# songlab-cal/CherryML

Measured on AMD Instinct MI355X. Metric: cherry-pairs/sec (whole node) per EM iter, higher is better.
Workload: dtype f64

## Files before the change

### cherryml_amd/csrc/cb_internal.hip.h

```cpp
#pragma once
#include "../../include/cherrybank.h"

#include <hip/hip_runtime.h>

#include <algorithm>
#include <atomic>
#include <chrono>
#include <cmath>
#include <cstdarg>
#include <cstdio>
#include <cstdlib>
#include <cstring>
#include <string>
#include <vector>

int cb_fail(int code, const char *fmt, ...);
#define fail cb_fail

#define HIP_TRY(expr)                                                                   \
  do {                                                                                  \
    hipError_t e_ = (expr);                                                             \
    if (e_ != hipSuccess)                                                               \
      return fail(e_ == hipErrorOutOfMemory ? CB_ENOMEM : CB_EHIP, "%s failed: %s (%s:%d)", \
                  #expr, hipGetErrorString(e_), __FILE__, __LINE__);                    \
  } while (0)

#define CB_REUSE_EIGH 256
int cb_internal_expm_bank(cb_handle h, const double *Q, const double *pi, int flags, double *P);
int cb_internal_set_times(cb_handle h, const double *t_host, int B, const double *t_dev);
struct CbSpectral {
  int S = 0, LD = 0;
  const double *A = nullptr, *U = nullptr, *lam = nullptr, *dsq = nullptr, *sigma = nullptr;
};
int cb_internal_spectral(cb_handle h, CbSpectral *out);

int cb_launch_bank_fused(int variant, int kg, const void *args, int grid, hipStream_t stream, hipEvent_t stop);

#define CB_TB_RS_MAX 24
#define CB_TB_RG_MAX 40
struct CbTimeBasisHost {
  int B = 0, ns = 0, nd = 0, ng = 0;
  double rho_max = 0.0;
  double res_s = 0.0, res_g = 0.0;
  std::vector<int> kind;
  std::vector<int> skel_s, direct, skel_g;
  std::vector<double> tf, tg;
  std::vector<double> Ls, Lg;
};
bool cb_tb_build(int B, const double *t, double rho_max, CbTimeBasisHost &out);
struct CbTbEwArgs {
  int S, LD, B, ns, nd, ng;
  int nsmall;
  const double *Ct;
  const double *Psi;
  const double *A;
  const double *t;
  const double *Ls, *Lg;
  double *Gh;
  float *Gh32;
  double *loss_part;
  double inv_n;
  const unsigned long long *skip;
};
int cb_tb_launch_tables(int LD, int ns, int nd, int ng, const double *tf, const double *tg, const double *lam, double *F, double *E,
                        double *H, const unsigned long long *skip, hipStream_t stream);
#define CB_TB_LDS_MAX (144u << 10)
size_t cb_tb_ew_lds_bytes(int B, int ns, int ng);
bool cb_tb_supported(int B, int LD, int ns, int ng);
int cb_tb_prepare_ew(int B, int ns, int ng, size_t *cache);
int cb_tb_launch_ew(const CbTbEwArgs &a, hipStream_t stream, hipEvent_t stop, int *nparts);

static inline const char *cb_test_hook(const char *name) {
  const char *on = getenv("CB_TEST_HOOKS");
  return (on && on[0] == '1') ? getenv(name) : nullptr;
}

struct CbDevBufs {
  std::vector<void *> ptrs;
  ~CbDevBufs() {
    for (void *p : ptrs)
      if (p) (void)hipFree(p);
  }
  template <typename T>
  T *up(const T *host, size_t count, int &rc) {
    void *q = nullptr;
    if (rc != CB_OK) return nullptr;
    if (hipMalloc(&q, (count ? count : 1) * sizeof(T)) != hipSuccess) {
      rc = fail(CB_ENOMEM, "device allocation failed");
      return nullptr;
    }
    ptrs.push_back(q);
    if (host && count && hipMemcpyAsync(q, host, count * sizeof(T), hipMemcpyHostToDevice, 0) != hipSuccess)
      rc = fail(CB_EHIP, "upload failed");
    return static_cast<T *>(q);
  }
};

struct __attribute__((visibility("hidden"))) CbKernelTimer {
  const bool on, owned;
  hipEvent_t ev0 = nullptr, ev1 = nullptr;
  explicit CbKernelTimer(bool on_) : on(on_), owned(true) {}
  CbKernelTimer(bool on_, hipEvent_t b0, hipEvent_t b1) : on(on_), owned(false), ev0(b0), ev1(b1) {}
  CbKernelTimer(const CbKernelTimer &) = delete;
  ~CbKernelTimer() { drop(); }
  void drop() {
    if (owned && ev0) (void)hipEventDestroy(ev0);
    if (owned && ev1) (void)hipEventDestroy(ev1);
    ev0 = ev1 = nullptr;
  }
  int create() {
    HIP_TRY(hipEventCreate(&ev0));
    HIP_TRY(hipEventCreate(&ev1));
    return CB_OK;
  }
  int begin(bool sync_first) {
    if (!on) return CB_OK;
    const int rc = owned ? create() : CB_OK;
    if (rc != CB_OK) return rc;
    if (sync_first) HIP_TRY(hipStreamSynchronize(0));
    HIP_TRY(hipEventRecord(ev0, 0));
    return CB_OK;
  }
  int end(double *ms) {
    if (!on) return CB_OK;
    float t = 0.f;
    HIP_TRY(hipEventRecord(ev1, 0));
    HIP_TRY(hipEventSynchronize(ev1));
    HIP_TRY(hipEventElapsedTime(&t, ev0, ev1));
    *ms = t;
    drop();
    return CB_OK;
  }
};
```

### cherryml_amd/csrc/cherrybank.hip

```cpp
#include "cb_internal.hip.h"

#include "common.hip.h"
#include "jacobi_block.hip.h"
#include "jacobi_wave.hip.h"
#include "large_bank.hip.h"
#include "small_bank.hip.h"
#include "train_small.hip.h"
#include "train_large.hip.h"
#include "general_small.hip.h"
#include "general_large.hip.h"
#include "eigh_planned.hip.h"

#define CB_ABI_VERSION 2

static thread_local std::string g_err;

int cb_fail(int code, const char *fmt, ...) {
  char buf[512];
  va_list ap;
  va_start(ap, fmt);
  vsnprintf(buf, sizeof buf, fmt, ap);
  va_end(ap);
  g_err = buf;
  return code;
// ... 131 lines not shown
static double tb_growth() {
  if (const char *g = cb_test_hook("CB_TB_TEST_GROWTH")) return std::max(1.0, atof(g));
  return CB_TB_GROWTH;
}
static void tb_drop_next(cb_bank *h) {
  if (h->tb_next_pending) (void)h->tb_next.get();
  h->tb_next_pending = false;
}
static int tb_install(cb_bank *h, int B, CbTimeBasisHost &&nb, double ms) {
  if (nb.B != B || !cb_tb_supported(B, h->LD, nb.ns, nb.ng) || (h->dtype == CB_MIXED && 2 * (nb.ns + nb.nd) > B) ||
      cb_tb_prepare_ew(B, nb.ns, nb.ng, h->tb_ew_lds) != 0) {
    h->tb_failed = true;
    h->tb = CbTimeBasisHost{};
    return CB_OK;
  }
  const int set = h->tb_set ^ 1;
  HIP_TRY(hipMemcpy(h->tb_Ls[set], nb.Ls.data(), nb.Ls.size() * sizeof(double), hipMemcpyHostToDevice));
  HIP_TRY(hipMemcpy(h->tb_Lg[set], nb.Lg.data(), nb.Lg.size() * sizeof(double), hipMemcpyHostToDevice));
  HIP_TRY(hipMemcpy(h->tb_tf[set], nb.tf.data(), nb.tf.size() * sizeof(double), hipMemcpyHostToDevice));
  HIP_TRY(hipMemcpy(h->tb_tg[set], nb.tg.data(), nb.tg.size() * sizeof(double), hipMemcpyHostToDevice));
  h->tb = std::move(nb);
  h->tb_set = set;
  ++h->tb_builds;
  if (getenv("CB_DEBUG"))
    fprintf(stderr, "[cherrybank] time basis %d: rho_max %.3f, %d skeleton + %d direct forward, %d gradient buckets of %d; residuals %.1e / %.1e; %.1f ms%s\n",
            h->tb_builds, h->tb.rho_max, h->tb.ns, h->tb.nd, h->tb.ng, B, h->tb.res_s, h->tb.res_g, ms, ms < 0.0 ? " (built beside the epochs)" : "");
  return CB_OK;
}
static int tb_rebuild(cb_bank *h, int B, double two_sigma) {
  if (!(two_sigma > 0.0) || !std::isfinite(two_sigma)) return fail(CB_ENUMERIC, "time basis: max |Q_ii| = %g", 0.5 * two_sigma);
  tb_drop_next(h);
  const auto t0 = std::chrono::steady_clock::now();
  CbTimeBasisHost nb;
  if (!cb_tb_build(B, h->t_live_host.data(), two_sigma * tb_growth(), nb)) nb = CbTimeBasisHost{};
  HIP_TRY(hipStreamSynchronize(h->stream));
  return tb_install(h, B, std::move(nb), std::chrono::duration<double, std::milli>(std::chrono::steady_clock::now() - t0).count());
}
#ifndef CB_TB_LEAD
#define CB_TB_LEAD 64
#endif
static int tb_maintain(cb_bank *h, int B, int epoch, double two_sigma, bool stale) {
  if (cb_test_hook("CB_TB_TEST_GROWTH")) {
    if (stale) return tb_rebuild(h, B, two_sigma);
    return CB_OK;
  }
  if (h->tb_failed) return CB_OK;
  if (stale || !tb_in_range(h, B, two_sigma)) {
    bool took = false;
    if (h->tb_next_pending) {
      CbTimeBasisHost nb = h->tb_next.get();
      h->tb_next_pending = false;
      int rc = tb_install(h, B, std::move(nb), -1.0);
      if (rc != CB_OK || h->tb_failed) return rc;
      took = true;
    }
    if ((stale && !took) || !tb_in_range(h, B, two_sigma)) return tb_rebuild(h, B, two_sigma);
    return CB_OK;
  }
  double warn = 1.6;
  int lead = CB_TB_LEAD;
  if (const char *w = cb_test_hook("CB_TB_TEST_WARN")) sscanf(w, "%lf %d", &warn, &lead);
  if (h->tb_next_pending && epoch >= h->tb_next_epoch) {
    CbTimeBasisHost nb = h->tb_next.get();
    h->tb_next_pending = false;
    int rc = tb_install(h, B, std::move(nb), -1.0);
    if (rc != CB_OK || h->tb_failed) return rc;
  }
  if (!h->tb_next_pending && !tb_in_range(h, B, two_sigma, warn)) {
    std::vector<double> t(h->t_live_host.begin(), h->t_live_host.begin() + B);
    const double rho = two_sigma * tb_growth();
    h->tb_next = std::async(std::launch::async, [t, rho, B]() {
      CbTimeBasisHost nb;
      if (!cb_tb_build(B, t.data(), rho, nb)) nb = CbTimeBasisHost{};
      return nb;
    });
    h->tb_next_pending = true;
    h->tb_next_epoch = epoch + lead;
  }
  return CB_OK;
}

struct LargeBankForm {
  bool tb = false;
  bool fused = false;
  bool accum = false;
  int kg = 1;
  int n_parts = 1;
  int tiles_k3 = 0;
  int test_no_claim = 0;
  double phi_delta = 0;
};

static LargeBankForm choose_large_form(const cb_bank *h, int B, bool Pd, bool want_grad, bool planned_now) {
  static const int streams = getenv("CB_BANK_STREAMS") ? std::min(4, std::max(1, atoi(getenv("CB_BANK_STREAMS")))) : 1;
  const char *tb_hook = cb_test_hook("CB_BANK_TB"), *fused_hook = cb_test_hook("CB_BANK_FUSED"),
             *unfused_hook = cb_test_hook("CB_BANK_UNFUSED"), *k3_hook = cb_test_hook("CB_BANK_K3"),
             *kg_hook = cb_test_hook("CB_BANK_KG"), *no_claim_hook = cb_test_hook("CB_BANK_TEST_NO_CLAIM"),
             *phi_z_hook = cb_test_hook("CB_PHI_Z");
  const int LD = h->LD, tm = (LD + LG_TM - 1) / LG_TM, tn = (LD + LG_TN - 1) / LG_TN;
  const bool f32 = h->dtype == CB_F32 && !Pd;
  LargeBankForm f;
  const bool form_hooks = fused_hook || unfused_hook || k3_hook || kg_hook || no_claim_hook;
  f.tb = h->sym_counts && !h->per_bucket_products && !h->tb_block && !h->tb_failed && !Pd && want_grad && h->tb_Ls[0] &&
         streams == 1 && (h->dtype == CB_F64 || h->dtype == CB_MIXED) &&
         (tb_hook ? atoi(tb_hook) != 0 : (!form_hooks && B >= CB_TB_MIN_B));
  if (f.tb && planned_now && h->tb.B != B) f.tb = false;
  {
    const size_t nb16 = (size_t)LD / 16, cap = (size_t)B * tm * tn;
    if (nb16 * (nb16 + 1) > cap) f.tb = false;
  }
  f.fused = !Pd && want_grad && !unfused_hook && streams == 1 && h->bank_queue && (fused_hook || B >= CB_BANK_FUSED_MIN_B);
  f.accum = h->sym_counts && !h->per_bucket_products && !Pd && want_grad && h->Yk && streams == 1 && h->dtype == CB_F64 &&
            (k3_hook ? atoi(k3_hook) == 0 : (B >= CB_BANK_SUM_FIRST_MIN_B && h->phi_delta >= 4e-3));
  f.tiles_k3 = f.accum ? 0 : h->sym_counts ? tn * (tn + 1) / 2 : tm * tn;
  f.phi_delta = h->phi_delta;
  if (phi_z_hook) f.phi_delta *= atof(phi_z_hook) / 0.1;
  f.kg = (B < CB_BANK_KG2_MAX_B && !f32) ? 2 : 1;
  if (kg_hook) f.kg = atoi(kg_hook) == 1 ? 1 : 2;
  if (Pd) f.kg = 1;
  if (streams > 1 && h->dtype == CB_F64 && !Pd && want_grad && B >= 4 * streams && !h->comm && !h->profile) f.n_parts = streams;
  f.test_no_claim = no_claim_hook ? 1 : 0;
  return f;
}

struct LargeCall {
  int B;
  const double *t;
  double inv_n;
  double *loss, *dQ, *Pd;
  bool dA_padded, planned_now;
  const unsigned long long *skipw;
  size_t LL;
  int tiles, tiles_k1;
};

template <typename T1, typename TG>
struct BankBufs {
  const T1 *Ut, *A, *F, *Ct;
  TG *Gt, *T;
  const TG *U;
  int variant;
};
template <typename T1, typename TG>
static BankBufs<T1, TG> bank_bufs(const cb_bank *h) {
  if constexpr (std::is_same_v<T1, float>) return {h->Utf, h->Af, h->Ff, h->Ct32, h->Gt32, h->T32, h->Uf, 1};
  else if constexpr (std::is_same_v<TG, float>) return {h->Vc, h->A, h->F, h->Ct, h->Gt32, h->T32, h->Uf, 2};
  else return {h->Vc, h->A, h->F, h->Ct, h->Gt, h->T, h->U, 0};
}
template <typename Fn>
static int with_format(const cb_bank *h, bool Pd, Fn &&fn) {
  if (!Pd && h->dtype == CB_F32) return fn(float{}, float{});
  if (!Pd && h->dtype == CB_MIXED) return fn(double{}, float{});
  return fn(double{}, double{});
}

template <typename Args>
static void launch_kg(int kg, void (*kern1)(Args), void (*kern2)(Args), dim3 grid, hipStream_t st, hipEvent_t ev, const Args &a) {
  if (kg == 2) LAUNCH_STOP(ev, kern2, grid, dim3(2 * LG4_THREADS), 0, st, a);
  else LAUNCH_STOP(ev, kern1, grid, dim3(LG4_THREADS), 0, st, a);
}
static void launch_cast_f32(cb_bank *h, const LargeCall &c, size_t nF) {
  hipLaunchKernelGGL(lg_cast_f32, dim3((unsigned)((std::max(c.LL, nF) + 255) / 256)), dim3(256), 0, h->stream, c.LL, nF, h->U,
                     h->Vc, h->A, h->F, h->Uf, h->Utf, h->Af, h->Ff);
}
static void launch_tables(cb_bank *h, const LargeCall &c) {
  hipLaunchKernelGGL(lg_tables<NoBankArgs>, dim3((unsigned)(((size_t)c.B * h->LD + 255) / 256)), dim3(256), 0, h->stream, h->LD,
                     c.B, c.t, h->lam, h->sigma, h->F, h->E, h->H, NoBankArgs{}, (NoBankArgs *)nullptr, 0);
}

static void enqueue_k4(cb_bank *h, const LargeCall &c, const unsigned long long *skip, hipEvent_t stop) {
  const int S = h->S, LD = h->LD;
  K4Args k4a{S, LD, h->Mt, h->Vc, h->X, nullptr, nullptr, nullptr};
  k4a.skip = skip;
  launch_sg(h, k4a, 0);
  K4Args k4b{S, LD, h->Vc, h->X, c.dQ, c.dA_padded ? nullptr : h->dsq, nullptr, nullptr};
  k4b.skip = skip;
  launch_sg(h, k4b, 0, 0.0, 0.0, nullptr, stop);
}

template <typename TG>
static int enqueue_tail(cb_bank *h, const LargeBankForm &f, const LargeCall &c, const TG *src, int nb, int nparts, int sym_ld,
                        hipEvent_t k3_stop) {
  const int LD = h->LD;
  const LossArgs la{h->loss_part, nparts, h->S, h->dsq, h->dirsum, c.inv_n, c.loss, c.skipw};
  const dim3 red_grid((unsigned)((c.LL + 255) / 256) + 1);
  if (f.accum) {
    hipLaunchKernelGGL(ky_reduce_loss<TG>, red_grid, dim3(256), 0, h->stream, src, YArgs{LD, c.B, c.t, h->E, h->Yk}, la);
    K4Args gl{h->S, LD, h->Yk, h->U, h->Lk, nullptr, nullptr, nullptr};
    gl.skip = c.skipw;
    gl.ystride = c.LL;
    launch_sg(h, gl, 0, 0.0, 0.0, nullptr, nullptr, 1 + CB_PHI_TERMS);
    LAUNCH_STOP(k3_stop, kphi_combine<CB_PHI_TERMS>, dim3((unsigned)((c.LL + 255) / 256)), dim3(256), 0, h->stream, LD, h->Lk,
                h->lam, f.phi_delta, h->Mt, c.skipw);
  } else {
    hipLaunchKernelGGL(k3_reduce_loss<TG>, red_grid, dim3(256), 0, h->stream, src, nb, c.LL, h->Mt, sym_ld, la);
  }
  enqueue_k4(h, c, c.skipw, stop_event(h, EV_K4));
  HIP_TRY(hipGetLastError());
  return CB_OK;
}

template <typename TG>
static int enqueue_tb_bank(cb_bank *h, const LargeBankForm &f, const LargeCall &c) {
  constexpr bool mixed = std::is_same_v<TG, float>;
  const CbTimeBasisHost &bas = h->tb;
  const int S = h->S, LD = h->LD, set = h->tb_set, nf = bas.ns + bas.nd, ng = bas.ng;
  const auto bb = bank_bufs<double, TG>(h);
  if (!c.planned_now && cb_tb_launch_tables(LD, bas.ns, bas.nd, ng, h->tb_tf[set], h->tb_tg[set], h->lam, h->F, h->E, h->H,
                                            c.skipw, h->stream) != 0)
    return fail(CB_EHIP, "tb_tables: launch failed");
  double *psi_buf = mixed ? reinterpret_cast<double *>(h->T32) : h->T;
  K1Args<double> k1{S, LD, nf, h->Vc, h->A, h->tb_tf[set], h->F, h->sigma, h->Ct, psi_buf, h->loss_part, c.inv_n, h->dsq, nullptr, c.skipw};
  LAUNCH_STOP(stop_event(h, EV_K1), (k1_pt_loss_gt<double, double, false, 1, true>), dim3(c.tiles_k1 * nf), dim3(LG4_THREADS), 0,
              h->stream, k1);
  const CbTbEwArgs ew{S, LD, c.B, bas.ns, bas.nd, ng, c.B - bas.nd, h->Ct, psi_buf, h->A, c.t, h->tb_Ls[set], h->tb_Lg[set], h->Gt,
                      mixed ? h->Gt32 : nullptr, h->loss_part, c.inv_n, c.skipw};
  int ew_parts = 0;
  if (cb_tb_launch_ew(ew, h->stream, stop_event(h, EV_K2), &ew_parts) != 0) return fail(CB_EHIP, "tb_ew: launch failed");
  if (mixed) launch_cast_f32(h, c, 0);
  const K2Args<TG> k2{LD, bb.Gt, bb.U, bb.T, c.skipw};
  const K3Args<TG> k3{LD, ng, bb.T, bb.U, h->tb_tg[set], h->lam, h->E, h->H, bb.Gt, 1, c.skipw};
  hipLaunchKernelGGL((k2_t_eq_g_u<TG, 1>), dim3(c.tiles * ng), dim3(LG4_THREADS), 0, h->stream, k2);
  LAUNCH_STOP(stop_event(h, EV_K3), (k3_w_phi<TG, 1>), dim3(c.tiles_k1 * ng), dim3(LG4_THREADS), 0, h->stream, k3);
  return enqueue_tail<TG>(h, f, c, bb.Gt, ng, ew_parts, LD, nullptr);
}

template <typename T1, typename TG>
static int enqueue_fused_bank(cb_bank *h, const LargeBankForm &f, const LargeCall &c) {
  const int S = h->S, LD = h->LD, B = c.B;
  const auto bb = bank_bufs<T1, TG>(h);
  const int total = B * (c.tiles_k1 + c.tiles + f.tiles_k3), grid = std::min(h->bank_slots / f.kg, total);
  const int sym = h->sym_counts ? 1 : 0;
  if (h->profile && h->profile_now) h->ev_rec[EV_K1] = h->ev_rec[EV_K2] = false;
  const hipEvent_t bank_stop = stop_event(h, EV_K3);
  static_assert(sizeof(K123Args<float, float>) == sizeof(K123Args<double, double>) &&
                sizeof(K123Args<double, float>) == sizeof(K123Args<double, double>), "one argument block for all");
  const K123Args<T1, TG> a{{S, LD, B, bb.Ut, bb.A, c.t, bb.F, h->sigma, bb.Ct, bb.Gt, h->loss_part, c.inv_n, h->dsq, nullptr, c.skipw},
                           {LD, bb.Gt, bb.U, bb.T, c.skipw},
                           {LD, B, bb.T, bb.U, c.t, h->lam, h->E, h->H, bb.Gt, sym, c.skipw},
                           {h->bank_queue, B, c.tiles_k1, c.tiles, f.tiles_k3, h->bank_claims, f.test_no_claim}};
  auto *dst = reinterpret_cast<K123Args<T1, TG> *>(h->bank_args);
  hipLaunchKernelGGL((lg_tables<K123Args<T1, TG>>), dim3((unsigned)(((size_t)B * LD + 255) / 256)), dim3(256), 0, h->stream, LD, B,
                     c.t, h->lam, h->sigma, h->F, h->E, h->H, a, dst, grid);
  if (std::is_same_v<TG, float>) launch_cast_f32(h, c, (size_t)B * LD);
  if (cb_launch_bank_fused(bb.variant, f.kg, dst, grid, h->stream, bank_stop) != 0) return fail(CB_EHIP, "k123_bank: launch failed");
  return enqueue_tail<TG>(h, f, c, f.accum ? bb.T : bb.Gt, B, B * c.tiles_k1, h->sym_counts ? LD : 0, nullptr);
}

template <typename T1, typename TG>
static int enqueue_split_bank(cb_bank *h, const LargeBankForm &f, const LargeCall &c) {
  const int S = h->S, LD = h->LD, B = c.B;
  const auto bb = bank_bufs<T1, TG>(h);
  launch_tables(h, c);
  if (std::is_same_v<TG, float>) launch_cast_f32(h, c, (size_t)B * LD);
  const K1Args<T1, TG> k1{S, LD, B, bb.Ut, bb.A, c.t, bb.F, h->sigma, bb.Ct, bb.Gt, h->loss_part, c.inv_n, h->dsq, c.Pd, c.skipw};
  const hipEvent_t ev_k1 = stop_event(h, EV_K1);
  if constexpr (std::is_same_v<TG, double>) {
    if (c.Pd) {
      LAUNCH_STOP(ev_k1, (k1_pt_loss_gt<double, double, true>), dim3(c.tiles_k1 * B), dim3(LG4_THREADS), 0, h->stream, k1);
      HIP_TRY(hipGetLastError());
      return CB_OK;
    }
  }
  launch_kg(f.kg, k1_pt_loss_gt<T1, TG, false, 1>, k1_pt_loss_gt<T1, TG, false, 2>, dim3(c.tiles_k1 * B), h->stream, ev_k1, k1);
  if (!c.dQ) {
    hipLaunchKernelGGL(lg_finish_loss, dim3(1), dim3(256), 0, h->stream, h->loss_part, B * c.tiles_k1, S, h->dsq, h->dirsum,
                       c.inv_n, c.loss);
    HIP_TRY(hipGetLastError());
    return CB_OK;
  }
  const K2Args<TG> k2{LD, bb.Gt, bb.U, bb.T, c.skipw};
  launch_kg(f.kg, k2_t_eq_g_u<TG, 1>, k2_t_eq_g_u<TG, 2>, dim3(c.tiles * B), h->stream, stop_event(h, EV_K2), k2);
  const hipEvent_t ev_k3 = stop_event(h, EV_K3);
  if (f.accum) return enqueue_tail<TG>(h, f, c, bb.T, B, B * c.tiles_k1, 0, ev_k3);
  const K3Args<TG> k3{LD, B, bb.T, bb.U, c.t, h->lam, h->E, h->H, bb.Gt, h->sym_counts ? 1 : 0, c.skipw};
  launch_kg(f.kg, k3_w_phi<TG, 1>, k3_w_phi<TG, 2>, dim3(f.tiles_k3 * B), h->stream, ev_k3, k3);
  return enqueue_tail<TG>(h, f, c, bb.Gt, B, B * c.tiles_k1, h->sym_counts ? LD : 0, nullptr);
}

static int enqueue_stream_split_bank(cb_bank *h, const LargeBankForm &f, const LargeCall &c) {
  const int S = h->S, LD = h->LD, B = c.B, n = f.n_parts;
  const size_t LL = c.LL;
  launch_tables(h, c);
  if (!h->ev_fork) HIP_TRY(hipEventCreateWithFlags(&h->ev_fork, hipEventDisableTiming));
  for (int p = 1; p < n; ++p)
    if (!h->xstream[p - 1]) {
      HIP_TRY(hipStreamCreateWithFlags(&h->xstream[p - 1], hipStreamNonBlocking));
      HIP_TRY(hipEventCreateWithFlags(&h->ev_join[p - 1], hipEventDisableTiming));
    }
  HIP_TRY(hipEventRecord(h->ev_fork, h->stream));
  for (int p = 1; p < n; ++p) HIP_TRY(hipStreamWaitEvent(h->xstream[p - 1], h->ev_fork, 0));
  for (int k = 1; k <= 3; ++k)
    for (int p = 0; p < n; ++p) {
      const int b0 = (int)((long)B * p / n), Bs = (int)((long)B * (p + 1) / n) - b0;
      const hipStream_t st = p ? h->xstream[p - 1] : h->stream;
      double *Gt = h->Gt + b0 * LL, *T = h->T + b0 * LL;
      if (k == 1) {
        K1Args<double> k1{S, LD, Bs, h->Vc, h->A, c.t + b0, h->F + (size_t)b0 * LD, h->sigma, h->Ct + b0 * LL, Gt,
                          h->loss_part + (size_t)b0 * c.tiles_k1, c.inv_n, h->dsq, nullptr};
        launch_kg(f.kg, k1_pt_loss_gt<double, double, false, 1>, k1_pt_loss_gt<double, double, false, 2>, dim3(c.tiles_k1 * Bs),
                  st, nullptr, k1);
// ... 394 lines not shown
```

### cherryml_amd/csrc/handle_host.hip.h

```cpp
#pragma once
#include <hip/hip_ext.h>
#include <future>
struct EighSlot {
  int cap = 12;
  int nsq = 0;
  int band_after = 0;
  int so = 0;
  int expect_run = 1, expect_order = 12, expect_sq = 2;
};
struct EighPlan {
  int lead_band = 1;
  int nslots = 0;
  EighSlot slot[EC_MAXREC];
};
struct cb_bank {
  int dev = 0, S = 0, L = 0, B = 0;
  int B_cap = 0;
  hipStream_t xstream[3] = {};
  hipEvent_t ev_fork = nullptr, ev_join[3] = {};
  int tr_epochs = 0;
  uint64_t tr_sig = 0;
  int last_form = 0;
  double tr_pow_b1 = 1.0, tr_pow_b2 = 1.0;
  int dtype = CB_F64;
  int LD = 0;
  bool large = false;
  hipStream_t own_stream = nullptr, stream = nullptr;
  std::vector<void *> allocs;
  std::vector<double> n_host;
  double *t = nullptr;
  double *Ct = nullptr;
  double *n_dev = nullptr;
  double *inv_n = nullptr;
  double *ones = nullptr;
  double *Cq = nullptr;
  int nq = 0;
  double *dirsum = nullptr;
  double *dirsum_g = nullptr;
  int Bl = 0;
  double *t_live = nullptr;
  int *nlive = nullptr;
  std::vector<int> nlive_host;
  double *Q = nullptr, *pi = nullptr, *loss = nullptr, *dQ = nullptr;
  int *status = nullptr;
  double *Gc2 = nullptr, *gx = nullptr;
  int last_light = 0;
  void *comm = nullptr;
  int (*allreduce)(const void *, void *, size_t, int, int, void *, hipStream_t) = nullptr;
  double *inv_n_global = nullptr;
  std::vector<double> n_global;
  bool expm_only = false;
  bool per_bucket_products = false;
  bool sym_counts = false;
  int spec_sweeps = 0;
  double *A = nullptr, *dsq = nullptr, *Gc = nullptr, *Vc = nullptr, *U = nullptr, *lam = nullptr,
         *sigma = nullptr, *F = nullptr, *E = nullptr, *H = nullptr, *Gt = nullptr, *T = nullptr,
         *Mt_part = nullptr, *Mt = nullptr, *X = nullptr, *loss_part = nullptr;
  float *Ct32 = nullptr, *Gt32 = nullptr, *T32 = nullptr, *Uf = nullptr, *Utf = nullptr, *Af = nullptr, *Ff = nullptr;
  unsigned long long *off_bits = nullptr;
  unsigned long long *poll = nullptr;
  unsigned long long poll_seq = 0;
  unsigned long long *ectl = nullptr, *epin = nullptr;
  double *epart = nullptr;
  bool begin_folded = false;
  double *sigma_home = nullptr;
  double *sigma2 = nullptr;
  unsigned long long eseq = 0;
  bool planned_unavailable = false;
  int planned_solves = 0, planned_stalls = 0;
  long long record_spins = 0;
  std::vector<double> epoch_seconds;
  EighPlan eplan;
  int k3_chunk = 0, k3_nchunks = 0;
  double *Yk = nullptr, *Lk = nullptr;
  double phi_delta = 0.0;
  unsigned int *bank_queue = nullptr;
  unsigned char *bank_args = nullptr;
  int bank_slots = 0;
  int bank_claims = 0;
  bool bank_fused = false;
  int bank_kg = 1;
  bool bank_accum = false;
  CbTimeBasisHost tb;
  int tb_set = 0;
  double *tb_Ls[2] = {}, *tb_Lg[2] = {}, *tb_tf[2] = {}, *tb_tg[2] = {};
  std::future<CbTimeBasisHost> tb_next;
  bool tb_next_pending = false;
  int tb_next_epoch = 0;
  size_t tb_ew_lds[4] = {0, 0, 0, 0};
  int tb_builds = 0, tb_stale_epochs = 0;
  bool tb_failed = false;
  bool tb_block = false;
  bool bank_tb = false;
  int last_sweeps = 0;
  double *gn_scratch = nullptr, *gn_partial = nullptr;
  int gn_nw = 0;
  struct {
    double *Qn = nullptr, *QT = nullptr, *colsum = nullptr, *alpha = nullptr, *R = nullptr, *RT = nullptr, *E = nullptr,
           *ET = nullptr, *G = nullptr, *GT = nullptr, *Xbar = nullptr, *lpart = nullptr;
    int *nsq = nullptr;
    int cap_slots = 0;
  } gl;
  std::vector<double> t_host, t_live_host;
  bool have_prev = false;
  double *ws_ptr[16] = {};
  size_t ws_cap[16] = {};
  char *pin = nullptr;
  size_t pin_cap = 0, pin_off = 0;
  bool profile = false;
  int profile_every = 1;
  bool profile_now = false;
  hipEvent_t ev[CB_T_COUNT + 1] = {};
  bool ev_rec[CB_T_COUNT + 1] = {};
  double t_sum[CB_T_COUNT] = {};
  int t_calls = 0;
  bool t_pending = false;
  hipEvent_t ev2[CB_T_COUNT + 1] = {};
  bool ev_rec2[CB_T_COUNT + 1] = {};
  bool t_pending2 = false;
};

static void swap_event_sets(cb_bank *h) {
  for (int i = 0; i <= CB_T_COUNT; ++i) {
    std::swap(h->ev[i], h->ev2[i]);
    std::swap(h->ev_rec[i], h->ev_rec2[i]);
  }
  std::swap(h->t_pending, h->t_pending2);
}

static void fold_pending(cb_bank *h);
enum { EV_START = 0, EV_EIGH, EV_K1, EV_K2, EV_K3, EV_K4, EV_SMALL, EV_END, EV_AR };
static void mark(cb_bank *h, int which) {
  if (!h->profile || !h->profile_now) return;
  if (!h->ev[which]) (void)hipEventCreate(&h->ev[which]);
  (void)hipEventRecord(h->ev[which], h->stream);
  h->ev_rec[which] = true;
}

static hipEvent_t stop_event(cb_bank *h, int which) {
  if (!h->profile || !h->profile_now) return nullptr;
  if (!h->ev[which] && hipEventCreate(&h->ev[which]) != hipSuccess) return nullptr;
  h->ev_rec[which] = true;
  return h->ev[which];
}
static void clear_marks(cb_bank *h) {
  if (h->profile && !h->profile_now) return;
  for (bool &b : h->ev_rec) b = false;
}
#define LAUNCH_STOP(ev, kernel, grid, block, shmem, stream, ...)                                              \
  do {                                                                                                        \
    hipEvent_t ev_ = (ev);                                                                                    \
    if (ev_) hipExtLaunchKernelGGL(kernel, grid, block, shmem, stream, nullptr, ev_, 0, __VA_ARGS__);         \
    else hipLaunchKernelGGL(kernel, grid, block, shmem, stream, __VA_ARGS__);                                 \
  } while (0)

template <typename T>
static int dev_alloc(cb_bank *h, T **p, size_t count) {
  void *q = nullptr;
  hipError_t e = hipMalloc(&q, count * sizeof(T) + 64);
  if (e != hipSuccess)
    return fail(CB_ENOMEM, "hipMalloc of %zu bytes failed: %s", count * sizeof(T),
                hipGetErrorString(e));
  h->allocs.push_back(q);
  *p = static_cast<T *>(q);
  return CB_OK;
}
#define ALLOC(ptr, count)                         \
  do {                                            \
    int rc_ = dev_alloc(h, &(ptr), (count));      \
    if (rc_ != CB_OK) return rc_;                 \
  } while (0)

// ... 51 lines not shown
```

### cherryml_amd/csrc/tbasis.hip.h

```cpp
#pragma once
#include "cb_internal.hip.h"
#include "common.hip.h"
#include <hip/hip_ext.h>

namespace tbasis {

typedef long double ld;

static inline ld g_phi2(ld x) {
  if (fabsl(x) < 0.5L) {
    ld p = 1.0L;
    for (int k = 24; k >= 3; --k) p = 1.0L + p * x / (ld)k;
    return 0.5L * p;
  }
  return (expm1l(x) - x) / (x * x);
}

static inline ld dot4(const ld *a, const ld *b, int n) {
  ld s0 = 0.0L, s1 = 0.0L, s2 = 0.0L, s3 = 0.0L;
  int i = 0;
  for (; i + 3 < n; i += 4) {
    s0 += a[i] * b[i];
    s1 += a[i + 1] * b[i + 1];
    s2 += a[i + 2] * b[i + 2];
    s3 += a[i + 3] * b[i + 3];
  }
  for (; i < n; ++i) s0 += a[i] * b[i];
  return (s0 + s1) + (s2 + s3);
}

static int id_rows(int B, int N, const std::vector<ld> &F, int Rmax, ld tol, std::vector<int> &skel, std::vector<ld> &L, ld &resid) {
  std::vector<ld> W(F), Q((size_t)Rmax * N, 0.0L), Cq((size_t)B * Rmax, 0.0L), q(N);
  skel.clear();
  ld scale = 0.0L;
  int R = 0;
  bool done = false;
  for (int r = 0; r <= Rmax; ++r) {
    int p = -1;
    ld best = -1.0L;
    for (int b = 0; b < B; ++b) {
      const ld *w = &W[(size_t)b * N];
      const ld s = dot4(w, w, N);
      if (s > best) best = s, p = b;
    }
    if (r == 0) scale = sqrtl(best);
    if (!(scale > 0.0L) || sqrtl(best) <= tol * scale) {
      done = true;
      break;
    }
    if (r == Rmax) break;
    const ld inv = 1.0L / sqrtl(best);
    for (int i = 0; i < N; ++i) q[i] = W[(size_t)p * N + i] * inv;
    for (int pass = 0; pass < 2; ++pass) {
      for (int k = 0; k < r; ++k) {
        const ld *qk = &Q[(size_t)k * N];
        const ld d = dot4(qk, q.data(), N);
        for (int i = 0; i < N; ++i) q[i] -= d * qk[i];
      }
      const ld s = dot4(q.data(), q.data(), N);
      const ld in = 1.0L / sqrtl(s);
      for (int i = 0; i < N; ++i) q[i] *= in;
    }
    for (int i = 0; i < N; ++i) Q[(size_t)r * N + i] = q[i];
    for (int b = 0; b < B; ++b) {
      ld *w = &W[(size_t)b * N];
      const ld c = dot4(w, q.data(), N);
      Cq[(size_t)b * Rmax + r] = c;
      for (int i = 0; i < N; ++i) w[i] -= c * q[i];
    }
    skel.push_back(p);
    R = r + 1;
  }
  if (!done) return -1;
  L.assign((size_t)B * std::max(R, 1), 0.0L);
  for (int r = R - 1; r >= 0; --r) {
    const ld trr = Cq[(size_t)skel[r] * Rmax + r];
    for (int b = 0; b < B; ++b) {
      ld s = Cq[(size_t)b * Rmax + r];
      for (int k = r + 1; k < R; ++k) s -= L[(size_t)b * R + k] * Cq[(size_t)skel[k] * Rmax + r];
      L[(size_t)b * R + r] = s / trr;
    }
  }
  for (int r = 0; r < R; ++r)
    for (int k = 0; k < R; ++k) L[(size_t)skel[r] * R + k] = k == r ? 1.0L : 0.0L;
  resid = 0.0L;
  for (int b = 0; b < B; ++b)
// ... 22 lines not shown
  out = CbTimeBasisHost{};
  if (B < 1 || !(rho_max > 0.0) || !std::isfinite(rho_max)) return false;
  for (int b = 0; b < B; ++b)
    if (!(t[b] > 0.0) || !std::isfinite(t[b])) return false;
  const int N = CB_TB_SAMPLES + 1;
  std::vector<ld> mu(N);
  mu[0] = 0.0L;
  for (int i = 1; i < N; ++i) mu[i] = -(ld)rho_max * powl(10.0L, -6.0L + 6.0L * (ld)(i - 1) / (ld)(N - 2));
  out.B = B;
  out.rho_max = rho_max;
  for (int b = 1; b < B; ++b)
    if (!(t[b] >= t[b - 1])) return false;
  out.kind.assign(B, -1);
  std::vector<int> small_idx;
  for (int b = 0; b < B; ++b) {
    if (t[b] * rho_max <= CB_TB_X_SMALL) small_idx.push_back(b);
    else {
      out.kind[b] = (int)out.direct.size();
      out.direct.push_back(b);
    }
  }
  out.Ls.assign((size_t)B * CB_TB_RS_MAX, 0.0);
  out.Lg.assign((size_t)B * CB_TB_RG_MAX, 0.0);
  const int nsm = (int)small_idx.size();
  if (nsm > 0) {
    std::vector<ld> F((size_t)nsm * N);
    for (int k = 0; k < nsm; ++k)
      for (int i = 0; i < N; ++i) F[(size_t)k * N + i] = mu[i] * mu[i] * g_phi2((ld)t[small_idx[k]] * mu[i]);
    std::vector<int> sk;
    std::vector<ld> L;
    ld res = 0.0L;
    const int R = id_rows(nsm, N, F, std::min(CB_TB_RS_MAX, nsm), 1e-17L, sk, L, res);
    if (R < 0) return false;
    out.ns = R;
    out.res_s = (double)res;
    for (int r = 0; r < R; ++r) out.skel_s.push_back(small_idx[sk[r]]);
    for (int k = 0; k < nsm; ++k)
      for (int r = 0; r < R; ++r) out.Ls[(size_t)small_idx[k] * CB_TB_RS_MAX + r] = (double)L[(size_t)k * R + r];
  }
  out.nd = (int)out.direct.size();
  {
    std::vector<ld> F((size_t)B * N);
    for (int b = 0; b < B; ++b)
      for (int i = 0; i < N; ++i) F[(size_t)b * N + i] = expl((ld)t[b] * mu[i]);
    std::vector<int> sk;
    std::vector<ld> L;
    ld res = 0.0L;
    const int R = id_rows(B, N, F, std::min(CB_TB_RG_MAX, B), CB_TB_TOL_G, sk, L, res);
    if (R < 0) return false;
    out.ng = R;
    out.res_g = (double)res;
    out.skel_g = sk;
    for (int b = 0; b < B; ++b)
      for (int r = 0; r < R; ++r)
        out.Lg[(size_t)b * CB_TB_RG_MAX + r] = (double)(L[(size_t)b * R + r] * (ld)t[b] / (ld)t[sk[r]]);
  }
  for (int r = 0; r < out.ns; ++r) out.tf.push_back(t[out.skel_s[r]]);
  for (int r = 0; r < out.nd; ++r) out.tf.push_back(t[out.direct[r]]);
  for (int r = 0; r < out.ng; ++r) out.tg.push_back(t[out.skel_g[r]]);
  return true;
}

__global__ void tb_tables(int LD, int ns, int nd, int ng, const double *__restrict__ tf, const double *__restrict__ tg,
                          const double *__restrict__ lam, double *__restrict__ F, double *__restrict__ E, double *__restrict__ H,
                          const unsigned long long *skip) {
  if (skip && *skip != 0ull) return;
  const int idx = blockIdx.x * blockDim.x + threadIdx.x;
  const int nf = ns + nd;
  if (idx >= (nf + ng) * LD) return;
  const int r = idx / LD, k = idx - r * LD;
  if (r < nf) {
    const double t = tf[r], x = t * lam[k];
    F[idx] = r < ns ? phi2(x) / (t * t) : exp(x);
  } else {
    const double x = tg[r - nf] * lam[k];
    E[idx - nf * LD] = exp(x);
    H[idx - nf * LD] = exp(0.5 * x);
  }
}

template <int RS, int RG>
struct TbEwLds {
  static constexpr int SS = RS + 1, SG = RG + 2;
  int BP, LS, LG, TT, LT, RED, TOTAL;
  __host__ __device__ explicit TbEwLds(int B) {
    BP = (B + 15) & ~15;
    LS = 0;
    LG = LS + BP * SS;
    TT = LG + BP * SG;
    LT = TT + BP;
    RED = LT + 256;
    TOTAL = RED + 16;
  }
};

template <int RS, int RG>
__device__ __forceinline__ void tb_ew_step(int b0, int j, int k, int nsm, const double *sLs, const double *sLg, const double *sT,
                                           const double *ltab, const double (&psi)[RS / 4], double a_e, double dl, double inv_n,
                                           const double (&c)[4], const double (&pd)[4], d4 (&D)[RG / 16], double &loss, int &bad) {
  typedef TbEwLds<RS, RG> Lds;
  const bool any_small = b0 < nsm, any_direct = b0 + 16 > nsm;
  double P[4];
  if (any_small) {
    d4 acc = {0.0, 0.0, 0.0, 0.0};
#ifndef TB_NO_FWD
#pragma unroll
    for (int q = 0; q < RS / 4; ++q) acc = mfma_f64(sLs[(b0 + j) * Lds::SS + 4 * q + k], psi[q], acc);
#endif
#pragma unroll
    for (int m = 0; m < 4; ++m) {
      const double t = sT[b0 + k + 4 * m];
      P[m] = fma(t, fma(t, acc[m], a_e), dl);
    }
    if (any_direct) {
#pragma unroll
      for (int m = 0; m < 4; ++m) P[m] = (b0 + k + 4 * m < nsm) ? P[m] : pd[m];
    }
  } else {
#pragma unroll
    for (int m = 0; m < 4; ++m) P[m] = pd[m];
  }
  double g[4];
#pragma unroll
  for (int m = 0; m < 4; ++m) {
    const double cv = c[m];
    bad |= (!(P[m] >= 1e-300) && cv != 0.0) ? 1 : 0;
    const double Pu = fmax(P[m], 1e-300);
#ifdef TB_NO_LOG
    loss = fma(-cv, Pu, loss);
    g[m] = (-cv * inv_n) * Pu;
#else
    loss = fma(-cv, fast_log_table_unchecked(Pu, ltab), loss);
    g[m] = (-cv * inv_n) * fast_rcp(Pu);
#endif
  }
#ifdef TB_NO_BWD
#pragma unroll
  for (int m = 0; m < 4; ++m) D[0][m] += g[m];
#else
#pragma unroll
  for (int m = 0; m < 4; ++m) {
    const double *w = sLg + (b0 + 4 * m + k) * Lds::SG + j;
#pragma unroll
    for (int q = 0; q < RG / 16; ++q) D[q] = mfma_f64(w[16 * q], g[m], D[q]);
  }
#endif
}

template <int RS, int RG, int NWAVE, bool SYM>
__global__ __launch_bounds__(NWAVE * 64, 4) void tb_ew(CbTbEwArgs a) {
  constexpr int NT = NWAVE * 64;
  typedef TbEwLds<RS, RG> Lds;
  extern __shared__ double smem[];
  if (a.skip && *a.skip != 0ull) return;
  const Lds o(a.B);
  double *sLs = smem + o.LS, *sLg = smem + o.LG, *sT = smem + o.TT, *ltab = smem + o.LT, *sred = smem + o.RED;
  const int tid = threadIdx.x;
  for (int i = tid; i < o.BP * RS; i += NT) {
    const int b = i / RS, r = i - b * RS;
    sLs[b * Lds::SS + r] = b < a.B ? a.Ls[(size_t)b * CB_TB_RS_MAX + r] : 0.0;
  }
  for (int i = tid; i < o.BP * RG; i += NT) {
    const int b = i / RG, r = i - b * RG;
    sLg[b * Lds::SG + r] = (b < a.B && r < CB_TB_RG_MAX) ? a.Lg[(size_t)b * CB_TB_RG_MAX + r] : 0.0;
  }
  for (int i = tid; i < o.BP; i += NT) sT[i] = i < a.B ? a.t[i] : 0.0;
  fast_log_table_fill(ltab, tid, NT);
  __syncthreads();
  const size_t LL = (size_t)a.LD * a.LD;
  const int wave = tid >> 6, lane = tid & 63, j = lane & 15, k = lane >> 4;
  size_t e;
  bool live;
  double lossw = 1.0;
  if (SYM) {
    const int nb = a.LD / 16, item = (int)blockIdx.x * NWAVE + wave, blk = item >> 4, rr = item & 15;
    int I = 0, rest = blk;
    while (I < nb && rest >= nb - I) {
      rest -= nb - I;
      ++I;
    }
    live = I < nb;
    const int J = I + rest;
    e = live ? ((size_t)(16 * I + rr) * a.LD + 16 * J + j) : 0;
    lossw = J > I ? 2.0 : 1.0;
  } else {
    e = ((size_t)blockIdx.x * NWAVE + wave) * 16 + j;
    live = e < LL;
  }
  const size_t ec = live ? e : 0;
  const int row = (int)(ec / a.LD), col = (int)(ec - (size_t)row * a.LD);
  const double *__restrict__ Psi = a.Psi + ec;
  double psi[RS / 4];
#pragma unroll
  for (int q = 0; q < RS / 4; ++q) psi[q] = (4 * q + k < a.ns) ? Psi[(size_t)(4 * q + k) * LL] : 0.0;
  const double a_e = a.A[ec], dl = row == col ? 1.0 : 0.0;
  d4 D[RG / 16];
#pragma unroll
  for (int q = 0; q < RG / 16; ++q) D[q] = d4{0.0, 0.0, 0.0, 0.0};
  double loss = 0.0;
  int bad = 0;
  const int nsm = a.nsmall, B = a.B;
  const unsigned plane = (unsigned)(LL * sizeof(double));
  const __amdgpu_buffer_rsrc_t rc = __builtin_amdgcn_make_buffer_rsrc(const_cast<double *>(a.Ct), 0, 0x7fffffff, 0x00027000);
  const __amdgpu_buffer_rsrc_t rp = __builtin_amdgcn_make_buffer_rsrc(const_cast<double *>(a.Psi + (size_t)a.ns * LL), 0, 0x7fffffff, 0x00027000);
  const int eoff = (int)(ec * sizeof(double));
  int voff[4];
#pragma unroll
  for (int m = 0; m < 4; ++m) voff[m] = (int)((unsigned)(k + 4 * m) * plane) + eoff;
  auto load = [&](int b0, double (&cc)[4], double (&pp)[4]) {
    if (b0 >= B) return;
#ifdef TB_NO_LOAD
    for (int m = 0; m < 4; ++m) cc[m] = 1.0 + b0 + m, pp[m] = 0.5;
    return;
#endif
    if (b0 + 16 <= B) {
#pragma unroll
      for (int m = 0; m < 4; ++m)
        cc[m] = __builtin_bit_cast(double, __builtin_amdgcn_raw_buffer_load_b64(rc, voff[m], (int)((unsigned)b0 * plane), 0));
      if (b0 >= nsm) {
#pragma unroll
        for (int m = 0; m < 4; ++m)
          pp[m] = __builtin_bit_cast(double, __builtin_amdgcn_raw_buffer_load_b64(rp, voff[m], (int)((unsigned)(b0 - nsm) * plane), 0));
        return;
      }
      if (b0 + 16 <= nsm) return;
    } else {
#pragma unroll
      for (int m = 0; m < 4; ++m) {
        const bool in = b0 + k + 4 * m < B;
        const double v = __builtin_bit_cast(double, __builtin_amdgcn_raw_buffer_load_b64(rc, in ? voff[m] + (int)((unsigned)b0 * plane) : eoff, 0, 0));
        cc[m] = in ? v : 0.0;
      }
    }
#pragma unroll
    for (int m = 0; m < 4; ++m) {
      const int b = b0 + k + 4 * m;
      const bool in = b >= nsm && b < B;
      const double v = __builtin_bit_cast(double, __builtin_amdgcn_raw_buffer_load_b64(rp, (int)((unsigned)(in ? b - nsm : 0) * plane) + eoff, 0, 0));
      pp[m] = in ? v : 1.0;
    }
  };
  double c0[4] = {0.0, 0.0, 0.0, 0.0}, c1[4] = {0.0, 0.0, 0.0, 0.0}, p0[4] = {1.0, 1.0, 1.0, 1.0}, p1[4] = {1.0, 1.0, 1.0, 1.0};
  load(0, c0, p0);
  for (int b0 = 0; b0 < B; b0 += 32) {
    load(b0 + 16, c1, p1);
    tb_ew_step<RS, RG>(b0, j, k, nsm, sLs, sLg, sT, ltab, psi, a_e, dl, a.inv_n, c0, p0, D, loss, bad);
    if (b0 + 16 >= B) break;
    load(b0 + 32, c0, p0);
    tb_ew_step<RS, RG>(b0 + 16, j, k, nsm, sLs, sLg, sT, ltab, psi, a_e, dl, a.inv_n, c1, p1, D, loss, bad);
  }
  if (live) {
    if (a.Gh32) {
      float *__restrict__ Gh = a.Gh32 + e;
#pragma unroll
      for (int q = 0; q < RG / 16; ++q)
#pragma unroll
        for (int r = 0; r < 4; ++r) {
          const int rr = 16 * q + k + 4 * r;
          if (rr < a.ng) Gh[(size_t)rr * LL] = (float)D[q][r];
        }
    } else {
      double *__restrict__ Gh = a.Gh + e;
#pragma unroll
      for (int q = 0; q < RG / 16; ++q)
#pragma unroll
        for (int r = 0; r < 4; ++r) {
          const int rr = 16 * q + k + 4 * r;
          if (rr < a.ng) Gh[(size_t)rr * LL] = D[q][r];
        }
    }
  } else {
    loss = 0.0;
    bad = 0;
  }
  if (bad) loss = NAN;
  loss = wave_sum(loss) * lossw;
  if (lane == 0) sred[wave] = loss;
  __syncthreads();
  if (tid == 0) {
    double s = 0.0;
    for (int w = 0; w < NWAVE; ++w) s += sred[w];
    a.loss_part[blockIdx.x] = s;
  }
}

template <typename T>
__global__ __launch_bounds__(256) void tb_mirror(int LD, T *__restrict__ Gh, const unsigned long long *skip) {
  __shared__ T tile[16][17];
  if (skip && *skip != 0ull) return;
  const int nb = LD / 16;
  int I = 0, rest = (int)blockIdx.x;
  while (rest >= nb - 1 - I) {
    rest -= nb - 1 - I;
    ++I;
  }
  const int J = I + 1 + rest, r = threadIdx.x >> 4, c = threadIdx.x & 15;
  T *G = Gh + (size_t)blockIdx.y * LD * LD;
  tile[r][c] = G[(size_t)(16 * I + r) * LD + 16 * J + c];
  __syncthreads();
  G[(size_t)(16 * J + r) * LD + 16 * I + c] = tile[c][r];
}

int cb_tb_launch_tables(int LD, int ns, int nd, int ng, const double *tf, const double *tg, const double *lam, double *F, double *E,
                        double *H, const unsigned long long *skip, hipStream_t stream) {
  const int n = (ns + nd + ng) * LD;
  hipLaunchKernelGGL(tb_tables, dim3((unsigned)((n + 255) / 256)), dim3(256), 0, stream, LD, ns, nd, ng, tf, tg, lam, F, E, H, skip);
  return hipGetLastError() == hipSuccess ? 0 : -1;
}

bool cb_tb_supported(int B, int LD, int ns, int ng) {
  return ns <= CB_TB_RS_MAX && ng <= CB_TB_RG_MAX && LD % 16 == 0 && cb_tb_ew_lds_bytes(B, ns, ng) <= CB_TB_LDS_MAX &&
         (double)(B + 32) * (double)LD * (double)LD * 8.0 < 2147483648.0;
}

size_t cb_tb_ew_lds_bytes(int B, int ns, int ng) {
  const int RS = ns <= 16 ? 16 : 24, RG = ng <= 32 ? 32 : 48;
  const int BP = (B + 15) & ~15;
  return ((size_t)BP * (RS + 1 + RG + 2 + 1) + 256 + 16) * sizeof(double);
}

int cb_tb_prepare_ew(int B, int ns, int ng, size_t *cache) {
#define TB_PREP(RS_, RG_, slot_)                                                                                         \
  do {                                                                                                                   \
    const size_t lds = (size_t)TbEwLds<RS_, RG_>(B).TOTAL * sizeof(double);                                              \
    if (lds > cache[slot_]) {                                                                                            \
      if (hipFuncSetAttribute(reinterpret_cast<const void *>(tb_ew<RS_, RG_, 8, true>), hipFuncAttributeMaxDynamicSharedMemorySize, (int)lds) != hipSuccess) { \
        (void)hipGetLastError();                                                                                         \
        return -1;                                                                                                       \
      }                                                                                                                  \
      cache[slot_] = lds;                                                                                                \
    }                                                                                                                    \
  } while (0)
  if (ns <= 16 && ng <= 32) TB_PREP(16, 32, 0);
  else if (ns <= 16) TB_PREP(16, 48, 1);
  else if (ng <= 32) TB_PREP(24, 32, 2);
  else TB_PREP(24, 48, 3);
#undef TB_PREP
  return 0;
}

int cb_tb_launch_ew(const CbTbEwArgs &a, hipStream_t stream, hipEvent_t stop, int *nparts) {
  if (!cb_tb_supported(a.B, a.LD, a.ns, a.ng)) return -1;
  const int nb = a.LD / 16, nblk = nb * (nb + 1) / 2;
  const unsigned grid = (unsigned)(nblk * 2);
  if (nparts) *nparts = (int)grid;
#define TB_GO(RS_, RG_)                                                                                                  \
  do {                                                                                                                   \
    const size_t lds = (size_t)TbEwLds<RS_, RG_>(a.B).TOTAL * sizeof(double);                                            \
    hipLaunchKernelGGL((tb_ew<RS_, RG_, 8, true>), dim3(grid), dim3(512), lds, stream, a);                               \
  } while (0)
  if (a.ns <= 16 && a.ng <= 32) TB_GO(16, 32);
  else if (a.ns <= 16) TB_GO(16, 48);
  else if (a.ng <= 32) TB_GO(24, 32);
  else TB_GO(24, 48);
#undef TB_GO
  if (nb > 1) {
    const dim3 mg((unsigned)(nb * (nb - 1) / 2), (unsigned)a.ng);
    if (a.Gh32) {
      if (stop) hipExtLaunchKernelGGL(tb_mirror<float>, mg, dim3(256), 0, stream, nullptr, stop, 0, a.LD, a.Gh32, a.skip);
      else hipLaunchKernelGGL(tb_mirror<float>, mg, dim3(256), 0, stream, a.LD, a.Gh32, a.skip);
    } else {
      if (stop) hipExtLaunchKernelGGL(tb_mirror<double>, mg, dim3(256), 0, stream, nullptr, stop, 0, a.LD, a.Gh, a.skip);
      else hipLaunchKernelGGL(tb_mirror<double>, mg, dim3(256), 0, stream, a.LD, a.Gh, a.skip);
    }
  } else if (stop) {
    (void)hipEventRecord(stop, stream);
  }
  return hipGetLastError() == hipSuccess ? 0 : -1;
}
```

Measured before the change: 1.555 billion.

## Fuse symmetric mirror write into tb_ew kernel via LDS-staged transpose

The elementwise time-basis kernel now writes the transposed (mirrored) off-diagonal block itself, staging its per-lane results through shared memory so the transposed stores coalesce. This replaces the separate tb_mirror launch, which reread the upper triangle from global memory and wrote the lower triangle. The cost is extra LDS staging, a barrier and transposed stores at the end of each block, and possibly a larger LDS reservation when ng*144 doubles exceeds the table size. A test hook keeps the old two-kernel path available.

```diff
diff --git a/cherryml_amd/csrc/cb_internal.hip.h b/cherryml_amd/csrc/cb_internal.hip.h
--- a/cherryml_amd/csrc/cb_internal.hip.h
+++ b/cherryml_amd/csrc/cb_internal.hip.h
@@ -67,8 +67,9 @@
 #define CB_TB_LDS_MAX (144u << 10)
 size_t cb_tb_ew_lds_bytes(int B, int ns, int ng);
 bool cb_tb_supported(int B, int LD, int ns, int ng);
+#define CB_TB_EW_SLOTS 8
 int cb_tb_prepare_ew(int B, int ns, int ng, size_t *cache);
-int cb_tb_launch_ew(const CbTbEwArgs &a, hipStream_t stream, hipEvent_t stop, int *nparts);
+int cb_tb_launch_ew(const CbTbEwArgs &a, hipStream_t stream, hipEvent_t stop, int *nparts, bool legacy_sym);
 
 static inline const char *cb_test_hook(const char *name) {
   const char *on = getenv("CB_TEST_HOOKS");
diff --git a/cherryml_amd/csrc/cherrybank.hip b/cherryml_amd/csrc/cherrybank.hip
--- a/cherryml_amd/csrc/cherrybank.hip
+++ b/cherryml_amd/csrc/cherrybank.hip
@@ -237,6 +237,7 @@
 
 struct LargeBankForm {
   bool tb = false;
+  bool tb_legacy_sym = false;
   bool fused = false;
   bool accum = false;
   int kg = 1;
@@ -251,7 +252,7 @@
   const char *tb_hook = cb_test_hook("CB_BANK_TB"), *fused_hook = cb_test_hook("CB_BANK_FUSED"),
              *unfused_hook = cb_test_hook("CB_BANK_UNFUSED"), *k3_hook = cb_test_hook("CB_BANK_K3"),
              *kg_hook = cb_test_hook("CB_BANK_KG"), *no_claim_hook = cb_test_hook("CB_BANK_TEST_NO_CLAIM"),
-             *phi_z_hook = cb_test_hook("CB_PHI_Z");
+             *phi_z_hook = cb_test_hook("CB_PHI_Z"), *tb_legacy_hook = cb_test_hook("CB_TB_LEGACY_SYM");
   const int LD = h->LD, tm = (LD + LG_TM - 1) / LG_TM, tn = (LD + LG_TN - 1) / LG_TN;
   const bool f32 = h->dtype == CB_F32 && !Pd;
   LargeBankForm f;
@@ -260,6 +261,7 @@
          streams == 1 && (h->dtype == CB_F64 || h->dtype == CB_MIXED) &&
          (tb_hook ? atoi(tb_hook) != 0 : (!form_hooks && B >= CB_TB_MIN_B));
   if (f.tb && planned_now && h->tb.B != B) f.tb = false;
+  f.tb_legacy_sym = tb_legacy_hook && atoi(tb_legacy_hook) != 0;
   {
     const size_t nb16 = (size_t)LD / 16, cap = (size_t)B * tm * tn;
     if (nb16 * (nb16 + 1) > cap) f.tb = false;
@@ -371,7 +373,7 @@
   const CbTbEwArgs ew{S, LD, c.B, bas.ns, bas.nd, ng, c.B - bas.nd, h->Ct, psi_buf, h->A, c.t, h->tb_Ls[set], h->tb_Lg[set], h->Gt,
                       mixed ? h->Gt32 : nullptr, h->loss_part, c.inv_n, c.skipw};
   int ew_parts = 0;
-  if (cb_tb_launch_ew(ew, h->stream, stop_event(h, EV_K2), &ew_parts) != 0) return fail(CB_EHIP, "tb_ew: launch failed");
+  if (cb_tb_launch_ew(ew, h->stream, stop_event(h, EV_K2), &ew_parts, f.tb_legacy_sym) != 0) return fail(CB_EHIP, "tb_ew: launch failed");
   if (mixed) launch_cast_f32(h, c, 0);
   const K2Args<TG> k2{LD, bb.Gt, bb.U, bb.T, c.skipw};
   const K3Args<TG> k3{LD, ng, bb.T, bb.U, h->tb_tg[set], h->lam, h->E, h->H, bb.Gt, 1, c.skipw};
diff --git a/cherryml_amd/csrc/handle_host.hip.h b/cherryml_amd/csrc/handle_host.hip.h
--- a/cherryml_amd/csrc/handle_host.hip.h
+++ b/cherryml_amd/csrc/handle_host.hip.h
@@ -87,7 +87,7 @@
   std::future<CbTimeBasisHost> tb_next;
   bool tb_next_pending = false;
   int tb_next_epoch = 0;
-  size_t tb_ew_lds[4] = {0, 0, 0, 0};
+  size_t tb_ew_lds[CB_TB_EW_SLOTS] = {};
   int tb_builds = 0, tb_stale_epochs = 0;
   bool tb_failed = false;
   bool tb_block = false;
diff --git a/cherryml_amd/csrc/tbasis.hip.h b/cherryml_amd/csrc/tbasis.hip.h
--- a/cherryml_amd/csrc/tbasis.hip.h
+++ b/cherryml_amd/csrc/tbasis.hip.h
@@ -2,6 +2,7 @@
 #include "cb_internal.hip.h"
 #include "common.hip.h"
 #include <hip/hip_ext.h>
+#include <mutex>
 
 namespace tbasis {
 
@@ -190,6 +191,7 @@
 template <int RS, int RG>
 struct TbEwLds {
   static constexpr int SS = RS + 1, SG = RG + 2;
+  static constexpr int ST = 16 * 9;
   int BP, LS, LG, TT, LT, RED, TOTAL;
   __host__ __device__ explicit TbEwLds(int B) {
     BP = (B + 15) & ~15;
@@ -198,6 +200,10 @@
     TT = LG + BP * SG;
     LT = TT + BP;
     RED = LT + 256;
+    TOTAL = RED + 16;
+  }
+  __host__ __device__ TbEwLds(int B, int stage_rows) : TbEwLds(B) {
+    if (stage_rows * ST > RED) RED = stage_rows * ST;
     TOTAL = RED + 16;
   }
 };
@@ -255,13 +261,14 @@
 #endif
 }
 
-template <int RS, int RG, int NWAVE, bool SYM>
-__global__ __launch_bounds__(NWAVE * 64, 4) void tb_ew(CbTbEwArgs a) {
+template <int RS, int RG, int NWAVE, bool SYM, bool MIR>
+__device__ __forceinline__ void tb_ew_body(const CbTbEwArgs &a) {
+  static_assert(!MIR || (SYM && NWAVE == 8), "half a block per workgroup: the staging area's layout");
   constexpr int NT = NWAVE * 64;
   typedef TbEwLds<RS, RG> Lds;
   extern __shared__ double smem[];
   if (a.skip && *a.skip != 0ull) return;
-  const Lds o(a.B);
+  const Lds o = MIR ? Lds(a.B, a.ng) : Lds(a.B);
   double *sLs = smem + o.LS, *sLg = smem + o.LG, *sT = smem + o.TT, *ltab = smem + o.LT, *sred = smem + o.RED;
   const int tid = threadIdx.x;
   for (int i = tid; i < o.BP * RS; i += NT) {
@@ -280,15 +287,16 @@
   size_t e;
   bool live;
   double lossw = 1.0;
+  int I = 0, J = 0;
   if (SYM) {
     const int nb = a.LD / 16, item = (int)blockIdx.x * NWAVE + wave, blk = item >> 4, rr = item & 15;
-    int I = 0, rest = blk;
+    int rest = blk;
     while (I < nb && rest >= nb - I) {
       rest -= nb - I;
       ++I;
     }
     live = I < nb;
-    const int J = I + rest;
+    J = I + rest;
     e = live ? ((size_t)(16 * I + rr) * a.LD + 16 * J + j) : 0;
     lossw = J > I ? 2.0 : 1.0;
   } else {
@@ -390,6 +398,38 @@
     for (int w = 0; w < NWAVE; ++w) s += sred[w];
     a.loss_part[blockIdx.x] = s;
   }
+  if constexpr (MIR) {
+    if (!live || J == I) return;
+    double *stage = smem;
+#pragma unroll
+    for (int q = 0; q < RG / 16; ++q)
+#pragma unroll
+      for (int r = 0; r < 4; ++r) {
+        const int rr = 16 * q + k + 4 * r;
+        if (rr < a.ng) stage[rr * Lds::ST + j * (NWAVE + 1) + wave] = D[q][r];
+      }
+    __syncthreads();
+    const int wc = tid & (NWAVE - 1), jr = (tid / NWAVE) & 15, half = (int)blockIdx.x & 1;
+    const size_t em = (size_t)(16 * J + jr) * a.LD + 16 * I + NWAVE * half + wc;
+    const double *src = stage + jr * (NWAVE + 1) + wc;
+    constexpr int PASS = NT / (16 * NWAVE);
+    if (a.Gh32) {
+      float *__restrict__ Gh = a.Gh32 + em;
+      for (int r = tid / (16 * NWAVE); r < a.ng; r += PASS) Gh[(size_t)r * LL] = (float)src[r * Lds::ST];
+    } else {
+      double *__restrict__ Gh = a.Gh + em;
+      for (int r = tid / (16 * NWAVE); r < a.ng; r += PASS) Gh[(size_t)r * LL] = src[r * Lds::ST];
+    }
+  }
+}
+
+template <int RS, int RG, int NWAVE, bool SYM>
+__global__ __launch_bounds__(NWAVE * 64, 4) void tb_ew(CbTbEwArgs a) {
+  tb_ew_body<RS, RG, NWAVE, SYM, false>(a);
+}
+template <int RS, int RG>
+__global__ __launch_bounds__(512, 4) void tb_ew_mir(CbTbEwArgs a) {
+  tb_ew_body<RS, RG, 8, true, true>(a);
 }
 
 template <typename T>
@@ -424,20 +464,37 @@
 size_t cb_tb_ew_lds_bytes(int B, int ns, int ng) {
   const int RS = ns <= 16 ? 16 : 24, RG = ng <= 32 ? 32 : 48;
   const int BP = (B + 15) & ~15;
-  return ((size_t)BP * (RS + 1 + RG + 2 + 1) + 256 + 16) * sizeof(double);
-}
-
+  const size_t tables = (size_t)BP * (RS + 1 + RG + 2 + 1) + 256, stage = (size_t)ng * 16 * 9;
+  return (std::max(tables, stage) + 16) * sizeof(double);
+}
+
+static int tb_raise_lds(const void *fn, int slot, size_t lds, size_t *cache) {
+  constexpr int MAXDEV = 64;
+  static size_t high[MAXDEV][8] = {};
+  static std::mutex lock;
+  if (lds <= cache[slot]) return 0;
+  int dev = 0;
+  if (hipGetDevice(&dev) != hipSuccess || dev < 0 || dev >= MAXDEV) {
+    (void)hipGetLastError();
+    return -1;
+  }
+  std::lock_guard<std::mutex> guard(lock);
+  const size_t want = std::max(lds, high[dev][slot]);
+  if (hipFuncSetAttribute(fn, hipFuncAttributeMaxDynamicSharedMemorySize, (int)want) != hipSuccess) {
+    (void)hipGetLastError();
+    return -1;
+  }
+  high[dev][slot] = cache[slot] = want;
+  return 0;
+}
 int cb_tb_prepare_ew(int B, int ns, int ng, size_t *cache) {
 #define TB_PREP(RS_, RG_, slot_)                                                                                         \
   do {                                                                                                                   \
-    const size_t lds = (size_t)TbEwLds<RS_, RG_>(B).TOTAL * sizeof(double);                                              \
-    if (lds > cache[slot_]) {                                                                                            \
-      if (hipFuncSetAttribute(reinterpret_cast<const void *>(tb_ew<RS_, RG_, 8, true>), hipFuncAttributeMaxDynamicSharedMemorySize, (int)lds) != hipSuccess) { \
-        (void)hipGetLastError();                                                                                         \
-        return -1;                                                                                                       \
-      }                                                                                                                  \
-      cache[slot_] = lds;                                                                                                \
-    }                                                                                                                    \
+    if (tb_raise_lds(reinterpret_cast<const void *>(tb_ew_mir<RS_, RG_>), slot_,                                         \
+                     (size_t)TbEwLds<RS_, RG_>(B, ng).TOTAL * sizeof(double), cache) != 0 ||                             \
+        tb_raise_lds(reinterpret_cast<const void *>(tb_ew<RS_, RG_, 8, true>), 4 + slot_,                                \
+                     (size_t)TbEwLds<RS_, RG_>(B).TOTAL * sizeof(double), cache) != 0)                                   \
+      return -1;                                                                                                         \
   } while (0)
   if (ns <= 16 && ng <= 32) TB_PREP(16, 32, 0);
   else if (ns <= 16) TB_PREP(16, 48, 1);
@@ -447,21 +504,25 @@
   return 0;
 }
 
-int cb_tb_launch_ew(const CbTbEwArgs &a, hipStream_t stream, hipEvent_t stop, int *nparts) {
+int cb_tb_launch_ew(const CbTbEwArgs &a, hipStream_t stream, hipEvent_t stop, int *nparts, bool legacy_sym) {
   if (!cb_tb_supported(a.B, a.LD, a.ns, a.ng)) return -1;
   const int nb = a.LD / 16, nblk = nb * (nb + 1) / 2;
   const unsigned grid = (unsigned)(nblk * 2);
   if (nparts) *nparts = (int)grid;
 #define TB_GO(RS_, RG_)                                                                                                  \
   do {                                                                                                                   \
+    const size_t lds_mir = (size_t)TbEwLds<RS_, RG_>(a.B, a.ng).TOTAL * sizeof(double);                                  \
     const size_t lds = (size_t)TbEwLds<RS_, RG_>(a.B).TOTAL * sizeof(double);                                            \
-    hipLaunchKernelGGL((tb_ew<RS_, RG_, 8, true>), dim3(grid), dim3(512), lds, stream, a);                               \
+    if (legacy_sym) hipLaunchKernelGGL((tb_ew<RS_, RG_, 8, true>), dim3(grid), dim3(512), lds, stream, a);               \
+    else if (stop) hipExtLaunchKernelGGL((tb_ew_mir<RS_, RG_>), dim3(grid), dim3(512), lds_mir, stream, nullptr, stop, 0, a); \
+    else hipLaunchKernelGGL((tb_ew_mir<RS_, RG_>), dim3(grid), dim3(512), lds_mir, stream, a);                           \
   } while (0)
   if (a.ns <= 16 && a.ng <= 32) TB_GO(16, 32);
   else if (a.ns <= 16) TB_GO(16, 48);
   else if (a.ng <= 32) TB_GO(24, 32);
   else TB_GO(24, 48);
 #undef TB_GO
+  if (!legacy_sym) return hipGetLastError() == hipSuccess ? 0 : -1;
   if (nb > 1) {
     const dim3 mg((unsigned)(nb * (nb - 1) / 2), (unsigned)a.ng);
     if (a.Gh32) {
```

New measurement: 1.567 billion (median of 4 runs). Within noise of the previous version (+0.8%).
